# wavelab/libwave

Measured on AMD Instinct MI355X. Metric: point-cloud registrations/sec (1M<->1M pts, ICP), higher is better.
Workload: dtype f32

## Files before the change

include/wavematch.h:

```cpp
#ifndef WAVEMATCH_H
#define WAVEMATCH_H

#include <stddef.h>
#include <stdint.h>

#ifdef __cplusplus
extern "C" {
#endif

#define WM_OK 0
#define WM_NOT_CONVERGED 1
#define WM_TOO_FEW_CORRESPONDENCES 2
#define WM_ERR_ARG (-1)
#define WM_ERR_HIP (-2)
#define WM_ERR_RCCL (-3)
#define WM_ERR_STATE (-4)
#define WM_ERR_NOMEM (-5)

enum { WM_MEM_HOST = 0, WM_MEM_DEVICE = 1 };

typedef struct wm_ctx wm_ctx;

int wm_ctx_create(wm_ctx **out, int device);
void wm_ctx_destroy(wm_ctx *ctx);
// ... 94 lines not shown
int wm_icp_batch_match(wm_ctx *ctx, const wm_batch_item *items, int n_items, size_t stride_bytes,
                       int mem, const wm_icp_params *p, float res, int multiscale_steps,
                       int with_info, double *T_out, double *info_out, wm_icp_stats *stats,
                       int *status);

int wm_voxel_downsample_batch(wm_ctx *ctx, const wm_batch_item *items, int n_items, size_t stride_bytes,
                              int mem, float leaf, float *out_xyz, size_t cap_points, size_t *n_out);

int wm_voxel_downsample(wm_ctx *ctx, const void *pts, size_t n, size_t stride_bytes, int mem,
                        float leaf, void *out, size_t out_stride, int out_mem, size_t cap,
                        size_t *n_out);

int wm_transform_cloud(wm_ctx *ctx, const void *pts, size_t n, size_t stride_bytes, int mem,
                       const double T[16], void *out, size_t out_stride, int out_mem);

enum { WM_INFO_LUM = 0, WM_INFO_CENSI = 1, WM_INFO_LUMOLD = 2 };
int wm_icp_info(wm_ctx *ctx, int method, const double T_result[16], double lin_covar,
                double ang_covar, double max_corr, double info[36], int *degenerate);

int wm_debug_copy_bandwidth(wm_ctx *ctx, size_t bytes, int reps, double *gb_per_s);
int wm_debug_bins_sum(const double *x, size_t n, const unsigned *perm, double *out, long long limbs_out[3]);
int wm_debug_sort_pairs(wm_ctx *ctx, const void *keys, int key_bytes, size_t n, unsigned bits, unsigned *values_out);
int wm_debug_knn(wm_ctx *ctx, int which, int k, int32_t *idx_out, float *d2_out);
int wm_set_option(wm_ctx *ctx, const char *name, double value);
int wm_debug_cert_log(wm_ctx *ctx, int iterations, unsigned *out, int cap);
int wm_debug_cert_prof(wm_ctx *ctx, unsigned long long *out, int cap);
int wm_debug_pub_log(wm_ctx *ctx, unsigned long long *out, int cap);
int wm_get_iteration_times(wm_ctx *ctx, float *nn_ms, int cap);

int wm_debug_solve_cycles(wm_ctx *ctx, unsigned long long out[8]);
int wm_debug_cost_log(wm_ctx *ctx, int iterations, unsigned *out, size_t cap);
int wm_debug_phase_log(wm_ctx *ctx, unsigned long long *out, int iterations);

int wm_get_correspondences(wm_ctx *ctx, int32_t *match_idx, float *d2, size_t cap);

int wm_nn_search(wm_ctx *ctx, const double T[16], double max_corr, int nn_method,
                 int32_t *match_idx, float *d2, size_t cap, float *kernel_ms);

int wm_estimate_normals(wm_ctx *ctx, int which, int k, void *normals_out, int out_mem);

#define WM_STATS_LEN 32
int wm_icp_stats_for(wm_ctx *ctx, const double T[16], int mode, double stats[WM_STATS_LEN]);

int wm_debug_rank_select(wm_ctx *ctx, const float *vals, size_t n, size_t rank, float *out);

typedef struct { int n_matched, n_kept; float threshold_d2; int all_kept; } wm_icp_reject_result;
// ... 343 lines not shown
```

libwave_amd/capi.py:

```python
import ctypes as C
import os

import numpy as np

_HERE = os.path.dirname(os.path.abspath(__file__))
LIB_PATH = os.path.join(_HERE, "libwavematch_hip.so")

WM_OK, WM_NOT_CONVERGED, WM_TOO_FEW = 0, 1, 2
WM_ERR_ARG, WM_ERR_HIP, WM_ERR_RCCL, WM_ERR_STATE, WM_ERR_NOMEM = -1, -2, -3, -4, -5
WM_NDT_BATCH_MAX_POINTS = 200000
WM_GICP_BATCH_MAX_POINTS = 100000
WM_BATCH_LDS_TARGET_POINTS = 10000
WM_BATCH_MAX_TARGET_POINTS = 65535
WM_GROUND_BATCH_MAX_KEYS = 0xFFFFFFFF
WM_GROUND_BATCH_MAX_POINTS = 0x7FFFFFF0
WM_MEM_HOST, WM_MEM_DEVICE = 0, 1
WM_ICP_SVD, WM_ICP_GN6, WM_ICP_PLANE = 0, 1, 2
WM_REJECT_NONE, WM_REJECT_TRIMMED, WM_REJECT_MEDIAN = 0, 1, 2
WM_NN_AUTO, WM_NN_GRID, WM_NN_BRUTE = 0, 1, 2
WM_NN_WARM = 0x100
WM_INFO_LUM, WM_INFO_CENSI, WM_INFO_LUMOLD = 0, 1, 2
WM_STATS_LEN = 32
CONV_NAMES = {0: "NOT_CONVERGED", 1: "ITERATIONS", 2: "TRANSFORM", 3: "ABS_MSE", 4: "REL_MSE",
              5: "NO_CORRESPONDENCES", 6: "FORCED", 7: "DEGENERATE"}
# ... 287 lines not shown
        L.wm_comm_world.argtypes = [C.c_void_p]
        L.wm_comm_mailboxes.argtypes = [C.c_void_p]
        L.wm_comm_set_exchange_timeout_ms.argtypes = [C.c_void_p, C.c_int]
        L.wm_icp_align_sharded.argtypes = [C.c_void_p, C.c_void_p, C.c_void_p, C.c_size_t, C.c_void_p,
                                           C.c_size_t, C.c_size_t, C.c_int, C.POINTER(IcpParams), _dp,
                                           C.POINTER(IcpStats)]
        L.wm_ndt_set_comm.argtypes = [C.c_void_p, C.c_void_p]
        L.wm_ndt_build_model.argtypes = [C.c_void_p, C.c_double]
        L.wm_set_source_filtered.argtypes = [C.c_void_p, C.c_void_p, C.c_size_t, C.c_size_t, C.c_int, C.c_float]
        L.wm_set_target_filtered.argtypes = [C.c_void_p, C.c_void_p, C.c_size_t, C.c_size_t, C.c_int, C.c_float]
        L.wm_multi_create.argtypes = [C.POINTER(C.c_void_p), C.POINTER(C.c_int), C.c_int, C.c_int]
        L.wm_multi_destroy.argtypes = [C.c_void_p]
        L.wm_multi_destroy.restype = None
        L.wm_multi_size.argtypes = [C.c_void_p]
        L.wm_multi_icp_align.argtypes = [C.c_void_p, C.c_void_p, C.c_size_t, C.c_void_p, C.c_size_t,
                                         C.c_size_t, C.POINTER(IcpParams), _dp, C.POINTER(IcpStats)]
        L.wm_multi_icp_match.argtypes = [C.c_void_p, C.c_void_p, C.c_size_t, C.c_void_p, C.c_size_t,
                                         C.c_size_t, C.POINTER(IcpParams), C.c_float, C.c_int, _dp, C.POINTER(IcpStats)]
        L.wm_multi_icp_info.argtypes = [C.c_void_p, C.c_int, _dp, C.c_double, C.c_double, C.c_double, _dp,
                                        C.POINTER(C.c_int)]
        L.wm_debug_solve_cycles.argtypes = [C.c_void_p, C.POINTER(C.c_uint64)]
        L.wm_debug_sort_pairs.argtypes = [C.c_void_p, C.c_void_p, C.c_int, C.c_size_t, C.c_uint, C.c_void_p]
        L.wm_debug_knn.argtypes = [C.c_void_p, C.c_int, C.c_int, _ip, _fp]
        L.wm_debug_cost_log.argtypes = [C.c_void_p, C.c_int, C.c_void_p, C.c_size_t]
        L.wm_debug_phase_log.argtypes = [C.c_void_p, C.c_void_p, C.c_int]
        L.wm_get_correspondences.argtypes = [C.c_void_p, _ip, _fp, C.c_size_t]
        L.wm_nn_search.argtypes = [C.c_void_p, _dp, C.c_double, C.c_int, _ip, _fp, C.c_size_t, _fp]
        L.wm_icp_stats_for.argtypes = [C.c_void_p, _dp, C.c_int, _dp]
        L.wm_debug_rank_select.argtypes = [C.c_void_p, _fp, C.c_size_t, C.c_size_t, _fp]
        L.wm_icp_reject.argtypes = [C.c_void_p, _dp, C.c_int, C.c_int, C.c_double, C.c_double, C.c_int,
                                    C.POINTER(IcpRejectResult), C.c_void_p, _dp]
        L.wm_estimate_normals.argtypes = [C.c_void_p, C.c_int, C.c_int, C.c_void_p, C.c_int]
        L.wm_umeyama_from_stats.argtypes = [_dp, _dp]
        L.wm_gn6_from_stats.argtypes = [_dp, _dp]
        L.wm_ground_default_params.argtypes = [C.POINTER(GroundParams)]
        L.wm_ground_default_params.restype = None
        L.wm_ground_segment.argtypes = [C.c_void_p, C.c_void_p, C.c_size_t, C.c_size_t, C.c_int,
                                        C.POINTER(GroundParams), C.c_int, C.c_void_p, C.c_size_t, C.c_int,
                                        C.POINTER(C.c_size_t), C.c_void_p, C.POINTER(GroundStats)]
        L.wm_ground_segment_batch.argtypes = [C.c_void_p, C.POINTER(GroundScan), C.c_int, C.c_size_t, C.c_int,
                                              C.POINTER(GroundParams), C.c_int, C.c_void_p, C.c_size_t, C.c_void_p,
                                              C.c_size_t, C.c_int, C.POINTER(C.c_size_t), C.c_void_p,
                                              C.POINTER(GroundStats), C.POINTER(C.c_float)]
        L.wm_outlier_default_params.argtypes = [C.POINTER(OutlierParams)]
        L.wm_outlier_default_params.restype = None
        L.wm_outlier_filter.argtypes = [C.c_void_p, C.c_void_p, C.c_size_t, C.c_size_t, C.c_int, C.POINTER(OutlierParams),
# ... 1055 lines not shown
    def phase_log_fetch(self, iterations):
        buf = np.zeros((iterations, 8), np.uint64)
        k = lib().wm_debug_phase_log(self._h, buf.ctypes.data_as(C.c_void_p), iterations)
        return buf[:max(k, 0)]

    def sort_pairs(self, keys, bits):
        keys = np.ascontiguousarray(keys)
        assert keys.dtype in (np.uint32, np.uint64) and keys.ndim == 1
        out = np.zeros(keys.shape[0], np.uint32)
        self._check(lib().wm_debug_sort_pairs(self._h, keys.ctypes.data, keys.dtype.itemsize, keys.shape[0], int(bits),
                                              out.ctypes.data), "wm_debug_sort_pairs")
        return out

    def debug_knn(self, which, k):
        n = self.n_tgt if which == 1 else self.n_src
        idx = np.full((n, int(k)), -1, np.int32)
        d2 = np.zeros((n, int(k)), np.float32)
        rc = self._check(lib().wm_debug_knn(self._h, int(which), int(k), idx.ctypes.data_as(_ip), d2.ctypes.data_as(_fp)),
                         "wm_debug_knn")
        if rc != WM_OK:
            raise WmError("wm_debug_knn: %s" % lib().wm_strerror(rc).decode())
        return idx, d2

    def solve_cycles(self):
        buf = (C.c_uint64 * 8)()
        lib().wm_debug_solve_cycles(self._h, buf)
        return [int(v) for v in buf]

    def iteration_times(self, cap=1024):
        buf = np.zeros(cap, np.float32)
        n = lib().wm_get_iteration_times(self._h, buf.ctypes.data_as(_fp), cap)
        return buf[:n].copy()

    def correspondences(self):
        idx = np.empty(self.n_src, np.int32)
        d2 = np.empty(self.n_src, np.float32)
        self._check(lib().wm_get_correspondences(self._h, idx.ctypes.data_as(_ip),
                                                 d2.ctypes.data_as(_fp), self.n_src),
                    "wm_get_correspondences")
        return idx, d2

    def nn_search(self, T=None, max_corr=3.0, nn_method=WM_NN_AUTO, want=True, timed=False):
        T = np.ascontiguousarray(np.eye(4) if T is None else T, np.float64)
        idx = np.empty(self.n_src, np.int32) if want else None
        d2 = np.empty(self.n_src, np.float32) if want else None
        ms = C.c_float(0)
# ... 177 lines not shown
```

libwave_amd/csrc/wm_ctx.hip:

```cpp
#include "wm_internal.hpp"

#include <float.h>
#include <stdlib.h>
#include <string.h>

#include <new>

namespace wm {

int prepare_work(wm_ctx *ctx) {
    const size_t n = ctx->n_src > 0 ? ctx->n_src : 1;
    WM_HIP(ctx, ctx->keys.reserve(n * sizeof(unsigned long long)));
    WM_HIP(ctx, ctx->match_pt.reserve(n * sizeof(float4)));
    WM_HIP(ctx, ctx->partials.reserve((n / 64 + 1024) * kAcc * sizeof(double)));
    WM_HIP(ctx, ctx->d_state.reserve(sizeof(IcpDevState)));
    if (!ctx->h_state)
        WM_HIP(ctx, hipHostMalloc((void **) &ctx->h_state, sizeof(IcpDevState), hipHostMallocDefault));
    return WM_OK;
}

bool use_brute(const wm_ctx *ctx, int nn_method) {
    if (nn_method == WM_NN_BRUTE) return true;
    if (nn_method == WM_NN_GRID) return false;
    return (double) ctx->n_src * (double) ctx->n_tgt_input <= 4.0e6;
// ... 164 lines not shown
    {"nn_balanced", "WM_TUNE_NN_BALANCED", &wm_ctx::tune_nn_balanced, nullptr, kIntMin, kIntMax, 0},
    {"lag", "WM_TUNE_LAG", &wm_ctx::tune_lag, nullptr, 1, 16, 0},
    {"spin_us", "WM_TUNE_SPIN_US", &wm_ctx::tune_spin_us, nullptr, kIntMin, kIntMax, 0},
    {"cert_from", "WM_TUNE_CERT_FROM", &wm_ctx::tune_cert_from, nullptr, kIntMin, kIntMax, 0},
    {"cert_disp", "WM_TUNE_CERT_DISP", nullptr, &wm_ctx::tune_cert_disp, 0, kFloatMax, kOpenLo},
    {"cert_changed", "WM_TUNE_CERT_CHANGED", nullptr, &wm_ctx::tune_cert_changed, 0, kFloatMax, kOpenLo},
    {"cert_unsettled", "WM_TUNE_CERT_UNSETTLED", nullptr, &wm_ctx::tune_cert_unsettled, 0, kFloatMax, kOpenLo},
    {"cert_pad_mul", "WM_TUNE_CERT_PAD_MUL", nullptr, &wm_ctx::tune_cert_pad_mul, 0, kFloatMax, 0},
    {"cert_pad_frac", "WM_TUNE_CERT_PAD_FRAC", nullptr, &wm_ctx::tune_cert_pad_frac, 0, kFloatMax, 0},
    {"late", "WM_TUNE_LATE", &wm_ctx::tune_late, nullptr, kIntMin, kIntMax, kFlag},
    {"bins", "WM_TUNE_BINS", &wm_ctx::tune_bins, nullptr, kIntMin, kIntMax, 0},
    {"early_source", "WM_TUNE_EARLY_SOURCE", &wm_ctx::tune_early_source, nullptr, kIntMin, kIntMax, 0},
    {"shard_force", "WM_SHARD_FORCE", &wm_ctx::tune_force_shard, nullptr, kIntMin, kIntMax, 0},
    {"trace", "WM_TRACE", &wm_ctx::trace, nullptr, kIntMin, kIntMax, kFlag},
    {"gicp_served", "WM_TUNE_GICP_SERVED", &wm_ctx::tune_gicp_served, nullptr, kIntMin, 2, kFlag},
    {"gicp_serve_test_stall_ms", "WM_TUNE_GICP_SERVE_TEST_STALL_MS", &wm_ctx::gicp_serve_test_stall_ms, nullptr, kIntMin, kIntMax, 0},
    {"gicp_blocks", "WM_TUNE_GICP_BLOCKS", &wm_ctx::tune_gicp_blocks, nullptr, 1, 4096, 0},
    {"knn_r0", "WM_TUNE_KNN_R0", nullptr, &wm_ctx::tune_knn_r0, 0.25, 8, kOrZero},
    {"gicp_profile", "WM_GICP_PROFILE", &wm_ctx::gicp_profile, nullptr, kIntMin, kIntMax, kFlag},
    {"outlier_cell_div", "WM_TUNE_OUTLIER_CELL_DIV", nullptr, &wm_ctx::tune_outlier_cell_div, 0.5, 8, 0},
    {"cluster_cell_div", "WM_TUNE_CLUSTER_CELL_DIV", nullptr, &wm_ctx::tune_cluster_cell_div, 0.5, 8, 0},
    {"sac_round", "WM_TUNE_SAC_ROUND", &wm_ctx::tune_sac_round, nullptr, 1, 1024, 0},
    {"radix_min", "WM_TUNE_RADIX_MIN", &wm_ctx::tune_radix_min, nullptr, kIntMin, kIntMax, 0},
    {"ndt_dense", "WM_TUNE_NDT_DENSE", &wm_ctx::tune_ndt_dense, nullptr, kIntMin, kIntMax, 0},
    {"ndt_vox_split", "WM_TUNE_NDT_VOX_SPLIT", &wm_ctx::tune_ndt_vox_split, nullptr, kIntMin, kIntMax, kNdtModel},
    {"ndt_keys64", "WM_TUNE_NDT_KEYS64", &wm_ctx::tune_ndt_keys64, nullptr, kIntMin, kIntMax, kFlag | kNdtModel},
    {"ndt_blocks", "WM_TUNE_NDT_BLOCKS", &wm_ctx::tune_ndt_blocks, nullptr, 0, 4096, 0},
    {"ndt_spec_hessian", "WM_TUNE_NDT_SPEC_HESSIAN", &wm_ctx::tune_ndt_spec_hessian, nullptr, kIntMin, kIntMax, 0},
    {"ndt_fused_fetch", "WM_TUNE_NDT_FUSED_FETCH", &wm_ctx::tune_ndt_fused_fetch, nullptr, kIntMin, kIntMax, 0},
    {"ndt_profile", "WM_NDT_PROFILE", &wm_ctx::ndt_profile, nullptr, kIntMin, kIntMax, kFlag},
};

int apply_option(wm_ctx *ctx, const Option &o, double v) {
    if ((o.flags & kFlag) && v != o.hi) v = v != 0 ? 1 : 0;
    if ((!(v >= o.lo && v <= o.hi) || ((o.flags & kOpenLo) && v == o.lo)) && !((o.flags & kOrZero) && v == 0)) return WM_ERR_ARG;
    if (o.i) ctx->*o.i = (int) v;
    else ctx->*o.f = (float) v;
    if (o.flags & kNdtModel) ctx->ndt_built = false;
    return WM_OK;
}
}

int wm_set_option(wm_ctx *ctx, const char *name, double value) {
    if (!ctx || !name) return WM_ERR_ARG;
    for (const Option &o : kOptions)
        if (strcmp(name, o.name) == 0) return apply_option(ctx, o, value);
// ... 31 lines not shown

int wm_ctx_set_stream(wm_ctx *ctx, void *hip_stream, int external) {
    if (!ctx) return WM_ERR_ARG;
    WM_HIP(ctx, hipSetDevice(ctx->device));
    WM_HIP(ctx, hipStreamSynchronize(ctx->stream));
    ctx->stream = external ? static_cast<hipStream_t>(hip_stream) : ctx->own_stream;
    return WM_OK;
}

void wm_ctx_destroy(wm_ctx *ctx) {
    if (!ctx) return;
    (void) hipSetDevice(ctx->device);
    if (ctx->stream) (void) hipStreamSynchronize(ctx->stream);
    DevBuf *bufs[] = {&ctx->src_sorted, &ctx->tgt_orig, &ctx->staging, &ctx->staging2, &ctx->cell_of, &ctx->counts,
                      &ctx->block_sums, &ctx->bbox_buf, &ctx->cloud_bbox, &ctx->keys, &ctx->keys_bak, &ctx->match_pt, &ctx->match_pt_bak, &ctx->d_levels, &ctx->ndt_keys, &ctx->ndt_keys2,
                      &ctx->ndt_vox, &ctx->ndt_vkey, &ctx->ndt_hkeys, &ctx->ndt_hvals, &ctx->ndt_dense, &ctx->ndt_meanf, &ctx->src_orig,
                      &ctx->gicp_c1, &ctx->gicp_c2, &ctx->gicp_mahal, &ctx->gicp_mailbox, &ctx->src_grid.pts,
                      &ctx->src_grid.cell_start, &ctx->vg_idx, &ctx->vg_idx2, &ctx->vg_perm,
                      &ctx->vg_perm2, &ctx->vg_tmp, &ctx->vg_seg, &ctx->io_a, &ctx->io_b, &ctx->ds_ref,
                      &ctx->ds_tgt, &ctx->match_ref, &ctx->match_tgt,
                      &ctx->partials, &ctx->partials2, &ctx->bins, &ctx->nn_bound, &ctx->late_ctl, &ctx->cert_count, &ctx->cert_prof, &ctx->cost_log, &ctx->phase_log, &ctx->shard_ref, &ctx->shard_tgt,
                      &ctx->shard_ref_band, &ctx->shard_tgt_band, &ctx->shard_misc, &ctx->shard_flags, &ctx->shard_pos_t,
                      &ctx->shard_pos_s, &ctx->shard_stats, &ctx->ndt_sum_dev, &ctx->corr_tmp_idx, &ctx->corr_tmp_d2, &ctx->d_state,
                      &ctx->plane_nrm, &ctx->plane_nrm_src, &ctx->plane_bins, &ctx->reject_buf, &ctx->reject_tmp};
    for (DevBuf *b : bufs) b->release();
    ctx->icp_stage.release();
    ctx->gicp_stage.release();
    ctx->ndt_stage.release();
    batch_voxel_release(ctx);
    ground_release(ctx);
    outlier_release(ctx);
    cluster_release(ctx);
    sac_release(ctx);
    boxes_release(ctx);
    fpfh_release(ctx);
    for (auto &l : ctx->levels) {
        l.pts.release();
        l.cell_start.release();
    }
    if (ctx->h_state) (void) hipHostFree(ctx->h_state);
    if (ctx->h_gicp) (void) hipHostFree(ctx->h_gicp);
    if (ctx->h_gicp_slots) (void) hipHostFree(ctx->h_gicp_slots);
    if (ctx->h_ndt) (void) hipHostFree(ctx->h_ndt);
    if (ctx->h_sig) (void) hipHostFree(ctx->h_sig);
    if (ctx->h_pub) (void) hipHostFree(ctx->h_pub);
    if (ctx->h_late) (void) hipHostFree(ctx->h_late);
    if (ctx->ev_block) (void) hipEventDestroy(ctx->ev_block);
// ... 102 lines not shown
```

libwave_amd/csrc/wm_debug.hip:

```cpp
#include "wm_internal.hpp"
#include "wm_bins.hpp"

#include <algorithm>
#include <vector>

#include <math.h>

namespace wm {

void late_debug_report(wm_ctx *ctx, unsigned late_blocks, int inside, int reason) {
    unsigned long long d[64 * 4];
    (void) hipStreamSynchronize(ctx->stream);
    if (hipMemcpy(d, (char *) ctx->late_ctl.p + late_ctl_bytes(), sizeof(d), hipMemcpyDeviceToHost) == hipSuccess) {
        fprintf(stderr, "[wm] late kernel: %d iterations, reason %d\n", inside, reason);
        for (int k = 0; k < inside && k < 64; ++k)
            fprintf(stderr, "  it %2d: workers (hand-out -> all rows in) %6.2f us | rows added %5.2f | solve %5.2f | hand-out %5.2f\n", k,
                    k ? ((long long) d[k * 4] - (long long) d[(k - 1) * 4 + 3]) * 0.01 : 0.0,
                    (d[k * 4 + 1] - d[k * 4]) * 0.01, (d[k * 4 + 2] - d[k * 4 + 1]) * 0.01,
                    (d[k * 4 + 3] - d[k * 4 + 2]) * 0.01);
        const int li = ctx->late_debug_iter;
        std::vector<unsigned long long> wst((size_t) late_blocks * 8);
        if (li >= 1 && li < inside && li < 64 && ctx->cert_prof.p &&
            hipMemcpy(wst.data(), ctx->cert_prof.p, wst.size() * 8, hipMemcpyDeviceToHost) == hipSuccess) {
            const unsigned long long t0 = d[(li - 1) * 4 + 3];
// ... 117 lines not shown
    for (int i = 0; i < n; ++i) {
        unsigned t = 0;
        for (int k = 0; k < 64; ++k) t += tmp[(size_t) i * 64 + k];
        out[i] = t;
    }
    return n;
}

int wm_debug_pub_log(wm_ctx *ctx, unsigned long long *out, int cap) {
    if (!ctx || !out || !ctx->h_pub) return WM_ERR_ARG;
    const int n = ctx->h_pub_slots < cap ? ctx->h_pub_slots : cap;
    for (int k = 0; k < n; ++k) out[k] = ctx->h_pub[k];
    return n;
}

int wm_debug_cert_prof(wm_ctx *ctx, unsigned long long *out, int cap) {
    if (!ctx || !out || !ctx->cert_prof.p) return WM_ERR_ARG;
    WM_HIP(ctx, hipSetDevice(ctx->device));
    const int n = ctx->cert_log_iter < cap ? ctx->cert_log_iter : cap;
    if (n > 0) WM_TRY(copy_to_caller(ctx, out, ctx->cert_prof.p, (size_t) n * 64 * sizeof(unsigned long long)));
    return n;
}

int wm_get_iteration_times(wm_ctx *ctx, float *nn_ms, int cap) {
    if (!ctx || !nn_ms || cap < 0) return 0;
    int n = (int) ctx->iter_nn_ms.size();
    if (n > cap) n = cap;
    for (int i = 0; i < n; ++i) nn_ms[i] = ctx->iter_nn_ms[i];
    return n;
}

}
```

libwave_amd/csrc/wm_grid.hip:

```cpp
#include <cstring>

#include <rocprim/rocprim.hpp>

#include "wm_internal.hpp"
#include "wm_sort.hpp"

#include <math.h>
#include <vector>
#include <string.h>

namespace wm {

__global__ void __launch_bounds__(kBlock) k_pack(const unsigned char *in, size_t n, size_t stride,
                                                  float4 *out) {
    size_t i = (size_t) blockIdx.x * kBlock + threadIdx.x;
    if (i >= n) return;
    const float *p = reinterpret_cast<const float *>(in + i * stride);
    float x = p[0], y = p[1], z = p[2];
    if (!(isfinite(x) && isfinite(y) && isfinite(z))) {
        x = y = z = __builtin_nanf("");
    }
    out[i] = make_float4(x, y, z, __uint_as_float((unsigned) i));
}

// ... 162 lines not shown
        for (int d = 0; d < 3; ++d) {
            out->lo[d] = lo[d];
            out->hi[d] = hi[d];
        }
}

int compute_bbox(wm_ctx *ctx, const float4 *pts, size_t n, Bbox *out, size_t *n_valid) {
    for (int d = 0; d < 3; ++d) out->lo[d] = out->hi[d] = 0.f;
    *n_valid = 0;
    if (n == 0) return WM_OK;
    float *res = (float *) pinned_scratch(ctx, 8 * sizeof(float) * kBboxBlocks);
    if (!res) return WM_ERR_HIP;
    WM_HIP(ctx, ctx->bbox_buf.reserve(8 * sizeof(float) * kBboxBlocks));
    unsigned blocks = 0;
    WM_TRY(launch_bbox(ctx, pts, n, ctx->bbox_buf.as<float>(), &blocks));
    WM_TRY(fast_fetch(ctx, res, ctx->bbox_buf.p, 8 * sizeof(float) * blocks));
    finish_bbox(res, blocks, out, n_valid);
    return WM_OK;
}

struct LinearKey {
    float ox, oy, oz, inv_h;
    int nx, ny, nz;
    __device__ unsigned operator()(const float4 &p) const {
        int cx = (int) floorf((p.x - ox) * inv_h);
        int cy = (int) floorf((p.y - oy) * inv_h);
        int cz = (int) floorf((p.z - oz) * inv_h);
        cx = min(max(cx, 0), nx - 1);
        cy = min(max(cy, 0), ny - 1);
        cz = min(max(cz, 0), nz - 1);
        return (unsigned) ((cz * ny + cy) * nx + cx);
    }
};

__device__ inline unsigned spread3(unsigned v) {
    v &= 0x3FFu;
    v = (v | (v << 16)) & 0x030000FFu;
    v = (v | (v << 8)) & 0x0300F00Fu;
    v = (v | (v << 4)) & 0x030C30C3u;
    v = (v | (v << 2)) & 0x09249249u;
    return v;
}

struct MortonKey {
    float ox, oy, oz, sx, sy, sz;
    int cells;
    __device__ unsigned operator()(const float4 &p) const {
        int cx = min(max((int) ((p.x - ox) * sx), 0), cells - 1);
        int cy = min(max((int) ((p.y - oy) * sy), 0), cells - 1);
        int cz = min(max((int) ((p.z - oz) * sz), 0), cells - 1);
        return spread3((unsigned) cx) | (spread3((unsigned) cy) << 1) |
               (spread3((unsigned) cz) << 2);
    }
};
// ... 52 lines not shown
    WM_HIP(ctx, hipGetLastError());
    return WM_OK;
}

template <class KeyFn>
static int counting_sort(wm_ctx *ctx, const float4 *pts, size_t n, KeyFn key, size_t ncells,
                         unsigned *cell_start , float4 *out) {
    WM_HIP(ctx, ctx->cell_of.reserve(2 * n * sizeof(unsigned)));
    WM_HIP(ctx, ctx->counts.reserve(ncells * sizeof(unsigned)));
    unsigned *counts = ctx->counts.as<unsigned>();
    unsigned *cell_of = ctx->cell_of.as<unsigned>(), *rank_of = cell_of + n;
    WM_HIP(ctx, hipMemsetAsync(counts, 0, ncells * sizeof(unsigned), ctx->stream));
    unsigned blocks = (unsigned) ((n + kBlock - 1) / kBlock);
    hipLaunchKernelGGL(HIP_KERNEL_NAME(k_count<KeyFn>), dim3(blocks), dim3(kBlock), 0, ctx->stream,
                       pts, n, key, cell_of, rank_of, counts);
    WM_HIP(ctx, hipGetLastError());
    WM_TRY(exclusive_scan(ctx, counts, ncells, cell_start));
    hipLaunchKernelGGL(k_scatter, dim3(blocks), dim3(kBlock), 0, ctx->stream, pts, n, cell_of, rank_of,
                       cell_start, out, ncells);
    WM_HIP(ctx, hipGetLastError());
    return WM_OK;
}

constexpr int kOccBlocks = 1024;
__global__ void __launch_bounds__(kBlock) k_count_occupied(const unsigned *cell_start,
                                                            size_t ncells, unsigned *out) {
    unsigned c = 0;
    for (size_t i = (size_t) blockIdx.x * kBlock + threadIdx.x; i < ncells;
         i += (size_t) gridDim.x * kBlock)
        c += (cell_start[i + 1] != cell_start[i]);
    for (int off = 32; off > 0; off >>= 1) c += __shfl_down(c, off);
    __shared__ unsigned s_c[kBlock / 64];
    if ((threadIdx.x & 63) == 0) s_c[threadIdx.x >> 6] = c;
    __syncthreads();
    if (threadIdx.x == 0) {
        for (int w = 1; w < kBlock / 64; ++w) c += s_c[w];
        out[blockIdx.x] = c;
    }
}

__global__ void k_pad_tail(const unsigned *cell_start, size_t ncells, float4 *pts) {
    const unsigned end = cell_start[ncells];
    const float nanv = __builtin_nanf("");
    if (threadIdx.x < 4) pts[end + threadIdx.x] = make_float4(nanv, nanv, nanv, __uint_as_float(kNoIdx));
}

static void grid_dims(const Bbox &bb, float h, int *nx, int *ny, int *nz) {
    *nx = (int) floor((bb.hi[0] - bb.lo[0]) / h) + 1;
    *ny = (int) floor((bb.hi[1] - bb.lo[1]) / h) + 1;
    *nz = (int) floor((bb.hi[2] - bb.lo[2]) / h) + 1;
}

int build_grid_level(wm_ctx *ctx, const float4 *pts, size_t n, const Bbox &bb, float h,
                     GridLevel *lvl, double *avg_occupancy) {
    int nx, ny, nz;
    grid_dims(bb, h, &nx, &ny, &nz);
    uint64_t ncells = (uint64_t) nx * ny * nz;
    lvl->ncells = ncells;
    WM_HIP(ctx, lvl->pts.reserve((n + 4) * sizeof(float4)));
    WM_HIP(ctx, lvl->cell_start.reserve((ncells + 1) * sizeof(unsigned)));
    LinearKey key{bb.lo[0], bb.lo[1], bb.lo[2], 1.0f / h, nx, ny, nz};
    if (n > 0) {
        WM_TRY(counting_sort(ctx, pts, n, key, ncells, lvl->cell_start.as<unsigned>(),
                             lvl->pts.as<float4>()));
    } else {
        WM_HIP(ctx, hipMemsetAsync(lvl->cell_start.p, 0, (ncells + 1) * sizeof(unsigned),
                                   ctx->stream));
        hipLaunchKernelGGL(k_pad_tail, dim3(1), dim3(64), 0, ctx->stream, lvl->cell_start.as<unsigned>(),
                           (size_t) ncells, lvl->pts.as<float4>());
    }
    float extent = fmaxf(fmaxf(bb.hi[0] - bb.lo[0], bb.hi[1] - bb.lo[1]), bb.hi[2] - bb.lo[2]);
    float amax = 0;
    for (int d = 0; d < 3; ++d) amax = fmaxf(amax, fmaxf(fabsf(bb.lo[d]), fabsf(bb.hi[d])));
    float ulp = fmaxf(amax, extent) * 1.2e-7f;
    lvl->d.ox = bb.lo[0];
    lvl->d.oy = bb.lo[1];
    lvl->d.oz = bb.lo[2];
    lvl->d.h = h;
    lvl->d.inv_h = 1.0f / h;
    lvl->d.slack = fmaxf(1e-3f, 8.0f * ulp / h);
    lvl->d.nx = nx;
    lvl->d.ny = ny;
    lvl->d.nz = nz;
    lvl->d.pts = lvl->pts.as<float4>();
    lvl->d.cell_start = lvl->cell_start.as<unsigned>();
// ... 106 lines not shown
    unsigned total = 0;
#pragma unroll
    for (int r = 0; r < 4; ++r) {
        unsigned s, e;
        child_run(fs, fnx, fny, fnz, X, Y, Z, r, &s, &e);
        total += e - s;
    }
    counts[c] = total;
}

__global__ void __launch_bounds__(kBlock)
    k_coarse_move(const unsigned *__restrict__ fs, const float4 *__restrict__ fpts, size_t fncells,
                  LinearKey key0, int shift, int fnx, int fny, int fnz, int cnx, int cny,
                  const unsigned *__restrict__ cs, float4 *__restrict__ out, size_t cncells) {
    const unsigned j = blockIdx.x * kBlock + threadIdx.x;
    if (j == 0) {
        const unsigned end = cs[(size_t) cncells];
        const float nanv = __builtin_nanf("");
#pragma unroll
        for (int u = 0; u < 4; ++u) out[end + u] = make_float4(nanv, nanv, nanv, __uint_as_float(kNoIdx));
    }
    if (j >= fs[fncells]) return;
    const float4 p = fpts[j];
    int x = min(max((int) floorf((p.x - key0.ox) * key0.inv_h), 0), key0.nx - 1) >> shift;
    int y = min(max((int) floorf((p.y - key0.oy) * key0.inv_h), 0), key0.ny - 1) >> shift;
    int z = min(max((int) floorf((p.z - key0.oz) * key0.inv_h), 0), key0.nz - 1) >> shift;
    const int X = x >> 1, Y = y >> 1, Z = z >> 1, r = (y & 1) + 2 * (z & 1);
    unsigned dst = cs[((size_t) Z * cny + Y) * cnx + X];
    for (int q = 0; q < r; ++q) {
        unsigned s, e;
        child_run(fs, fnx, fny, fnz, X, Y, Z, q, &s, &e);
        dst += e - s;
    }
    unsigned s, e;
    child_run(fs, fnx, fny, fnz, X, Y, Z, r, &s, &e);
    out[dst + (j - s)] = p;
}

static int derive_grid_level(wm_ctx *ctx, const GridLevel &fine, int fine_index, GridLevel *lvl,
                             size_t n) {
    const GridDev &f = fine.d;
    const int nx = (f.nx + 1) / 2, ny = (f.ny + 1) / 2, nz = (f.nz + 1) / 2;
    const uint64_t ncells = (uint64_t) nx * ny * nz;
    lvl->ncells = ncells;
    WM_HIP(ctx, lvl->pts.reserve((n + 4) * sizeof(float4)));
    WM_HIP(ctx, lvl->cell_start.reserve((ncells + 1) * sizeof(unsigned)));
    WM_HIP(ctx, ctx->counts.reserve(ncells * sizeof(unsigned)));
    unsigned *counts = ctx->counts.as<unsigned>();
    const unsigned blocks = (unsigned) ((ncells + kBlock - 1) / kBlock);
// ... 139 lines not shown
```

libwave_amd/csrc/wm_internal.hpp:

```cpp
#pragma once
#include <stdio.h>

#include <hip/hip_runtime.h>
#include <stdint.h>

#include <chrono>
#include <string>
#include <thread>
#include <vector>

#include "../../include/wavematch.h"
#include "wm_math.hpp"

namespace wm {

constexpr int kMaxLevels = 6;
constexpr int kBlock = 256;
constexpr unsigned kNoIdx = 0xFFFFFFFFu;
constexpr int kBlkLen = 34;
constexpr int kAcc = 18;

#define WM_HIP(ctx, call)                                                              \
    do {                                                                               \
        hipError_t _e = (call);                                                        \
// ... 211 lines not shown
    float tune_r_light = 16.0f;
    int tune_xcd_chunk = 32;
    int tune_nn_balanced = 1;
    int tune_lag = 2;
    int tune_spin_us = 80;
    int tune_bins = 1;
    int tune_early_source = 2;
    int tune_force_shard = 0;
    int tune_cert_from = -1;
    float tune_cert_disp = 0.15f;
    float tune_cert_changed = 0.05f;
    float tune_cert_unsettled = 0.40f;
    float tune_cert_pad_mul = 8.f, tune_cert_pad_frac = 0.5f;
    int tune_late = 0;
    int tune_gicp_served = 1;
    int gicp_serve_test_stall_ms = 0;
    int tune_gicp_blocks = 256;
    float tune_knn_r0 = 0.f;
    int gicp_profile = 0;
    float tune_outlier_cell_div = 2.f;
    float tune_cluster_cell_div = 2.f;
    int tune_sac_round = 256;
    int tune_radix_min = 256 << 10;
    int tune_ndt_dense = 2;
    int tune_ndt_vox_split = -1;
    int tune_ndt_keys64 = 0;
    int tune_ndt_blocks = 0;
    int tune_ndt_spec_hessian = 1;
    int tune_ndt_fused_fetch = 1;
    int ndt_profile = 0;
    int late_debug_iter = -1;
    bool cert_prof_on = false;
    std::string gicp_trace_path;
    bool gicp_serve_debug = false;
    int gicp_small_trace = 0;

    double tuned_h = 0, tuned_vol = 0;
    size_t tuned_n = 0;
    double tuned_src_h = 0, tuned_src_vol = 0;
    unsigned tuned_src_uses = 0;
    size_t tuned_src_n = 0;

    wm::DevBuf staging, staging2, cell_of, counts, block_sums, bbox_buf;
    wm::DevBuf match_pt, match_pt_bak;
    wm::PairStage icp_stage, gicp_stage, ndt_stage;
    void *batch_voxel = nullptr;
    void *ground = nullptr;
    void *outlier = nullptr;
    void *cluster = nullptr;
    void *sac = nullptr;
    void *boxes = nullptr;
    void *fpfh = nullptr;
    wm::DevBuf phase_log;
    wm::DevBuf cost_log;
    int cost_log_iter = 0, cost_log_cap = 0;
    wm::DevBuf keys, partials, partials2, corr_tmp_idx, corr_tmp_d2, d_levels;
    wm::LevelsDev levels_dev{};
    wm::DevBuf bins;
    bool bins_dirty = false;
    wm::DevBuf nn_bound;
    wm::DevBuf cert_count;
    wm::DevBuf cert_prof;
    int cert_log_iter = 0, cert_log_cap = 0;
    int cert_launches = 0;
    int late_capacity = 0;
    wm::DevBuf late_ctl;
// ... 260 lines not shown
```

Measured before the change: 294.3.

## Build grid levels with a two-pass row-band counting sort

Adds a new grid-construction path that first bins points into bands of (z,y) rows using per-tile LDS histograms, scans them, and scatters points into band order. A per-band kernel then does a cell-level counting sort in LDS to produce cell_start and the sorted points. The goal is to replace the global per-cell counting sort with LDS-local atomics, reducing global atomics and scan work over large cell counts. It is enabled by default through tune_grid_rows=1 when the grid shape and size fit the limits, and it costs an extra temporary buffer plus an extra pass over the points. A debug API for dumping grid levels is also added.

```diff
diff --git a/include/wavematch.h b/include/wavematch.h
--- a/include/wavematch.h
+++ b/include/wavematch.h
@@ -140,6 +140,8 @@
 int wm_debug_bins_sum(const double *x, size_t n, const unsigned *perm, double *out, long long limbs_out[3]);
 int wm_debug_sort_pairs(wm_ctx *ctx, const void *keys, int key_bytes, size_t n, unsigned bits, unsigned *values_out);
 int wm_debug_knn(wm_ctx *ctx, int which, int k, int32_t *idx_out, float *d2_out);
+int wm_debug_grid_level(wm_ctx *ctx, int level, double max_corr, float geom[5], int dims[3], size_t *n_points,
+                        unsigned *cell_start, size_t cell_cap, float *pts, size_t pts_cap);
 int wm_set_option(wm_ctx *ctx, const char *name, double value);
 int wm_debug_cert_log(wm_ctx *ctx, int iterations, unsigned *out, int cap);
 int wm_debug_cert_prof(wm_ctx *ctx, unsigned long long *out, int cap);
diff --git a/libwave_amd/capi.py b/libwave_amd/capi.py
--- a/libwave_amd/capi.py
+++ b/libwave_amd/capi.py
@@ -333,6 +333,8 @@
         L.wm_debug_solve_cycles.argtypes = [C.c_void_p, C.POINTER(C.c_uint64)]
         L.wm_debug_sort_pairs.argtypes = [C.c_void_p, C.c_void_p, C.c_int, C.c_size_t, C.c_uint, C.c_void_p]
         L.wm_debug_knn.argtypes = [C.c_void_p, C.c_int, C.c_int, _ip, _fp]
+        L.wm_debug_grid_level.argtypes = [C.c_void_p, C.c_int, C.c_double, _fp, _ip, C.POINTER(C.c_size_t), C.c_void_p,
+                                          C.c_size_t, C.c_void_p, C.c_size_t]
         L.wm_debug_cost_log.argtypes = [C.c_void_p, C.c_int, C.c_void_p, C.c_size_t]
         L.wm_debug_phase_log.argtypes = [C.c_void_p, C.c_void_p, C.c_int]
         L.wm_get_correspondences.argtypes = [C.c_void_p, _ip, _fp, C.c_size_t]
@@ -1434,6 +1436,20 @@
             raise WmError("wm_debug_knn: %s" % lib().wm_strerror(rc).decode())
         return idx, d2
 
+    def debug_grid_level(self, level, max_corr=0.0):
+        geom = np.zeros(5, np.float32)
+        dims = np.zeros(3, np.int32)
+        n = C.c_size_t(0)
+        args = (self._h, int(level), float(max_corr), geom.ctypes.data_as(_fp), dims.ctypes.data_as(_ip), C.byref(n))
+        self._check(lib().wm_debug_grid_level(*args, None, 0, None, 0), "wm_debug_grid_level")
+        ncells = int(dims[0]) * int(dims[1]) * int(dims[2])
+        cell_start = np.zeros(ncells + 1, np.uint32)
+        pts = np.zeros((n.value + 4, 4), np.float32)
+        self._check(lib().wm_debug_grid_level(*args, cell_start.ctypes.data, cell_start.size, pts.ctypes.data, pts.shape[0]),
+                    "wm_debug_grid_level")
+        return dict(origin=geom[:3].copy(), h=geom[3], inv_h=geom[4], dims=tuple(int(d) for d in dims),
+                    cell_start=cell_start, pts=pts)
+
     def solve_cycles(self):
         buf = (C.c_uint64 * 8)()
         lib().wm_debug_solve_cycles(self._h, buf)
diff --git a/libwave_amd/csrc/wm_ctx.hip b/libwave_amd/csrc/wm_ctx.hip
--- a/libwave_amd/csrc/wm_ctx.hip
+++ b/libwave_amd/csrc/wm_ctx.hip
@@ -210,6 +210,7 @@
     {"cluster_cell_div", "WM_TUNE_CLUSTER_CELL_DIV", nullptr, &wm_ctx::tune_cluster_cell_div, 0.5, 8, 0},
     {"sac_round", "WM_TUNE_SAC_ROUND", &wm_ctx::tune_sac_round, nullptr, 1, 1024, 0},
     {"radix_min", "WM_TUNE_RADIX_MIN", &wm_ctx::tune_radix_min, nullptr, kIntMin, kIntMax, 0},
+    {"grid_rows", "WM_TUNE_GRID_ROWS", &wm_ctx::tune_grid_rows, nullptr, 0, 2, 0},
     {"ndt_dense", "WM_TUNE_NDT_DENSE", &wm_ctx::tune_ndt_dense, nullptr, kIntMin, kIntMax, 0},
     {"ndt_vox_split", "WM_TUNE_NDT_VOX_SPLIT", &wm_ctx::tune_ndt_vox_split, nullptr, kIntMin, kIntMax, kNdtModel},
     {"ndt_keys64", "WM_TUNE_NDT_KEYS64", &wm_ctx::tune_ndt_keys64, nullptr, kIntMin, kIntMax, kFlag | kNdtModel},
@@ -287,7 +288,8 @@
                       &ctx->partials, &ctx->partials2, &ctx->bins, &ctx->nn_bound, &ctx->late_ctl, &ctx->cert_count, &ctx->cert_prof, &ctx->cost_log, &ctx->phase_log, &ctx->shard_ref, &ctx->shard_tgt,
                       &ctx->shard_ref_band, &ctx->shard_tgt_band, &ctx->shard_misc, &ctx->shard_flags, &ctx->shard_pos_t,
                       &ctx->shard_pos_s, &ctx->shard_stats, &ctx->ndt_sum_dev, &ctx->corr_tmp_idx, &ctx->corr_tmp_d2, &ctx->d_state,
-                      &ctx->plane_nrm, &ctx->plane_nrm_src, &ctx->plane_bins, &ctx->reject_buf, &ctx->reject_tmp};
+                      &ctx->plane_nrm, &ctx->plane_nrm_src, &ctx->plane_bins, &ctx->reject_buf, &ctx->reject_tmp,
+                      &ctx->row_hist, &ctx->row_tmp};
     for (DevBuf *b : bufs) b->release();
     ctx->icp_stage.release();
     ctx->gicp_stage.release();
diff --git a/libwave_amd/csrc/wm_debug.hip b/libwave_amd/csrc/wm_debug.hip
--- a/libwave_amd/csrc/wm_debug.hip
+++ b/libwave_amd/csrc/wm_debug.hip
@@ -163,6 +163,28 @@
     return n;
 }
 
+int wm_debug_grid_level(wm_ctx *ctx, int level, double max_corr, float geom[5], int dims[3], size_t *n_points,
+                        unsigned *cell_start, size_t cell_cap, float *pts, size_t pts_cap) {
+    if (!ctx || level < 0 || level >= kMaxLevels || !geom || !dims || !n_points) return WM_ERR_ARG;
+    if (ctx->n_tgt_input == 0) return WM_ERR_STATE;
+    WM_HIP(ctx, hipSetDevice(ctx->device));
+    if (max_corr > 0) {
+        WM_TRY(finalize_clouds(ctx));
+        WM_TRY(ensure_levels(ctx, max_corr));
+    }
+    if (level >= ctx->n_levels || !ctx->levels[level].built) return WM_ERR_STATE;
+    const GridLevel &l = ctx->levels[level];
+    geom[0] = l.d.ox, geom[1] = l.d.oy, geom[2] = l.d.oz, geom[3] = l.d.h, geom[4] = l.d.inv_h;
+    dims[0] = l.d.nx, dims[1] = l.d.ny, dims[2] = l.d.nz;
+    unsigned total = 0;
+    WM_TRY(copy_to_caller(ctx, &total, l.cell_start.as<unsigned>() + l.ncells, sizeof(unsigned)));
+    *n_points = total;
+    if ((cell_start && cell_cap < l.ncells + 1) || (pts && pts_cap < (size_t) total + 4)) return WM_ERR_ARG;
+    if (cell_start) WM_TRY(copy_to_caller(ctx, cell_start, l.cell_start.p, (l.ncells + 1) * sizeof(unsigned)));
+    if (pts) WM_TRY(copy_to_caller(ctx, pts, l.pts.p, ((size_t) total + 4) * sizeof(float4)));
+    return WM_OK;
+}
+
 int wm_get_iteration_times(wm_ctx *ctx, float *nn_ms, int cap) {
     if (!ctx || !nn_ms || cap < 0) return 0;
     int n = (int) ctx->iter_nn_ms.size();
diff --git a/libwave_amd/csrc/wm_grid.hip b/libwave_amd/csrc/wm_grid.hip
--- a/libwave_amd/csrc/wm_grid.hip
+++ b/libwave_amd/csrc/wm_grid.hip
@@ -208,14 +208,21 @@
 struct LinearKey {
     float ox, oy, oz, inv_h;
     int nx, ny, nz;
+    __device__ void cell(const float4 &p, int *cx, int *cy, int *cz) const {
+        *cx = min(max((int) floorf((p.x - ox) * inv_h), 0), nx - 1);
+        *cy = min(max((int) floorf((p.y - oy) * inv_h), 0), ny - 1);
+        *cz = min(max((int) floorf((p.z - oz) * inv_h), 0), nz - 1);
+    }
+    __device__ void row_x(const float4 &p, unsigned *row, unsigned *cx) const {
+        int x, y, z;
+        cell(p, &x, &y, &z);
+        *row = (unsigned) (z * ny + y);
+        *cx = (unsigned) x;
+    }
     __device__ unsigned operator()(const float4 &p) const {
-        int cx = (int) floorf((p.x - ox) * inv_h);
-        int cy = (int) floorf((p.y - oy) * inv_h);
-        int cz = (int) floorf((p.z - oz) * inv_h);
-        cx = min(max(cx, 0), nx - 1);
-        cy = min(max(cy, 0), ny - 1);
-        cz = min(max(cz, 0), nz - 1);
-        return (unsigned) ((cz * ny + cy) * nx + cx);
+        unsigned row, cx;
+        row_x(p, &row, &cx);
+        return row * (unsigned) nx + cx;
     }
 };
 
@@ -314,6 +321,183 @@
     return WM_OK;
 }
 
+constexpr int kRowThreads = 512;
+constexpr int kRowTile = kRowThreads * 8;
+constexpr unsigned kRowNxCap = 4000;
+constexpr unsigned kRowCounterWords = 16000;
+constexpr unsigned kRowBandRows = 8;
+constexpr unsigned kRowMaxBands = 8192;
+constexpr uint64_t kRowMaxTable = 1ull << 22;
+
+__device__ __forceinline__ unsigned rows_lds_scan(unsigned *a, unsigned n, unsigned *s_wave) {
+    const unsigned tid = threadIdx.x, lane = tid & 63u, wave = tid >> 6;
+    const unsigned per = (n + kRowThreads - 1) / kRowThreads;
+    const unsigned b = min(tid * per, n), e = min(b + per, n);
+    unsigned sum = 0;
+    for (unsigned i = b; i < e; ++i) sum += a[i];
+    const unsigned incl = wave_incl_scan(sum, lane);
+    if (lane == 63u) s_wave[wave] = incl;
+    __syncthreads();
+    unsigned run = incl - sum, all = 0;
+    for (unsigned w = 0; w < (unsigned) (kRowThreads / 64); ++w) {
+        if (w < wave) run += s_wave[w];
+        all += s_wave[w];
+    }
+    for (unsigned i = b; i < e; ++i) {
+        const unsigned v = a[i];
+        a[i] = run;
+        run += v;
+    }
+    __syncthreads();
+    return all;
+}
+
+__global__ void __launch_bounds__(kRowThreads) k_rows_hist(const float4 *__restrict__ pts, unsigned n, LinearKey key, unsigned rshift,
+                                                            unsigned bands, unsigned tiles, unsigned *__restrict__ hist) {
+    extern __shared__ unsigned s_mem[];
+    const unsigned tid = threadIdx.x, tile = blockIdx.x;
+    for (unsigned b = tid; b < bands; b += kRowThreads) s_mem[b] = 0u;
+    __syncthreads();
+    float4 p[8];
+#pragma unroll
+    for (unsigned r = 0; r < 8u; ++r) {
+        const unsigned i = tile * (unsigned) kRowTile + r * kRowThreads + tid;
+        p[r] = i < n ? pts[i] : make_float4(NAN, 0.f, 0.f, 0.f);
+    }
+#pragma unroll
+    for (unsigned r = 0; r < 8u; ++r)
+        if (p[r].x == p[r].x) {
+            unsigned row, cx;
+            key.row_x(p[r], &row, &cx);
+            atomicAdd(&s_mem[row >> rshift], 1u);
+        }
+    __syncthreads();
+    for (unsigned b = tid; b < bands; b += kRowThreads) hist[(size_t) b * tiles + tile] = s_mem[b];
+}
+
+__global__ void __launch_bounds__(kRowThreads) k_rows_scatter(const float4 *__restrict__ pts, unsigned n, LinearKey key, unsigned rshift,
+                                                               unsigned bands, unsigned tiles, const unsigned *__restrict__ hist,
+                                                               const unsigned *__restrict__ totals, unsigned *__restrict__ band_start,
+                                                               float4 *__restrict__ tmp) {
+    extern __shared__ unsigned s_mem[];
+    __shared__ unsigned s_wave[kRowThreads / 64];
+    const unsigned tid = threadIdx.x, tile = blockIdx.x;
+    float4 p[8];
+#pragma unroll
+    for (unsigned r = 0; r < 8u; ++r) {
+        const unsigned i = tile * (unsigned) kRowTile + r * kRowThreads + tid;
+        p[r] = i < n ? pts[i] : make_float4(NAN, 0.f, 0.f, 0.f);
+    }
+    for (unsigned b = tid; b < bands; b += kRowThreads) s_mem[b] = totals[b];
+    __syncthreads();
+    const unsigned all = rows_lds_scan(s_mem, bands, s_wave);
+    if (tile == 0) {
+        for (unsigned b = tid; b < bands; b += kRowThreads) band_start[b] = s_mem[b];
+        if (tid == 0) band_start[bands] = all;
+    }
+    for (unsigned b = tid; b < bands; b += kRowThreads) s_mem[b] += hist[(size_t) b * tiles + tile];
+    __syncthreads();
+#pragma unroll
+    for (unsigned r = 0; r < 8u; ++r)
+        if (p[r].x == p[r].x) {
+            unsigned row, cx;
+            key.row_x(p[r], &row, &cx);
+            tmp[atomicAdd(&s_mem[row >> rshift], 1u)] = p[r];
+        }
+}
+
+__global__ void __launch_bounds__(kRowThreads) k_rows_finish(const float4 *__restrict__ tmp, const unsigned *__restrict__ band_start,
+                                                              LinearKey key, unsigned nrows, unsigned rshift,
+                                                              unsigned *__restrict__ cell_start, float4 *__restrict__ out) {
+    extern __shared__ unsigned s_mem[];
+    __shared__ unsigned s_wave[kRowThreads / 64];
+    const unsigned nx = (unsigned) key.nx, tid = threadIdx.x;
+    const unsigned r0 = blockIdx.x << rshift;
+    const unsigned cells = min(1u << rshift, nrows - r0) * nx;
+    const unsigned s = band_start[blockIdx.x], e = band_start[blockIdx.x + 1];
+    for (unsigned k = tid; k < cells; k += kRowThreads) s_mem[k] = 0u;
+    __syncthreads();
+    for (unsigned j0 = s + tid; j0 < e; j0 += 4u * kRowThreads) {
+        float4 p[4];
+#pragma unroll
+        for (unsigned u = 0; u < 4u; ++u) {
+            const unsigned j = j0 + u * kRowThreads;
+            p[u] = j < e ? tmp[j] : make_float4(NAN, 0.f, 0.f, 0.f);
+        }
+#pragma unroll
+        for (unsigned u = 0; u < 4u; ++u)
+            if (j0 + u * kRowThreads < e) {
+                unsigned row, cx;
+                key.row_x(p[u], &row, &cx);
+                atomicAdd(&s_mem[min((row - r0) * nx + cx, cells - 1u)], 1u);
+            }
+    }
+    __syncthreads();
+    if (e != s) rows_lds_scan(s_mem, cells, s_wave);
+    unsigned *cs = cell_start + (size_t) r0 * nx;
+    for (unsigned k = tid; k < cells; k += kRowThreads) cs[k] = s + s_mem[k];
+    if (blockIdx.x == gridDim.x - 1 && tid == 0) {
+        cs[cells] = e;
+        const float nanv = __builtin_nanf("");
+#pragma unroll
+        for (int u = 0; u < 4; ++u) out[e + u] = make_float4(nanv, nanv, nanv, __uint_as_float(kNoIdx));
+    }
+    __syncthreads();
+    for (unsigned j0 = s + tid; j0 < e; j0 += 4u * kRowThreads) {
+        float4 p[4];
+#pragma unroll
+        for (unsigned u = 0; u < 4u; ++u) {
+            const unsigned j = j0 + u * kRowThreads;
+            p[u] = j < e ? tmp[j] : make_float4(NAN, 0.f, 0.f, 0.f);
+        }
+#pragma unroll
+        for (unsigned u = 0; u < 4u; ++u)
+            if (j0 + u * kRowThreads < e) {
+                unsigned row, cx;
+                key.row_x(p[u], &row, &cx);
+                out[s + atomicAdd(&s_mem[min((row - r0) * nx + cx, cells - 1u)], 1u)] = p[u];
+            }
+    }
+}
+
+constexpr unsigned kRowMinRows = 2048, kRowMinPoints = 32768;
+static bool rows_apply(int option, int nx, int ny, int nz, size_t n, unsigned *rshift) {
+    if (option == 0 || n == 0 || (unsigned) nx > kRowNxCap) return false;
+    const uint64_t nrows = (uint64_t) ny * nz;
+    unsigned sh = 0;
+    while ((2u << sh) <= kRowBandRows && (2u << sh) * (unsigned) nx <= kRowCounterWords) ++sh;
+    while (((nrows - 1) >> sh) + 1 > kRowMaxBands && (2u << sh) * (unsigned) nx <= kRowCounterWords) ++sh;
+    const uint64_t bands = ((nrows - 1) >> sh) + 1, tiles = (n + kRowTile - 1) / kRowTile;
+    if (bands > kRowMaxBands || bands * tiles > kRowMaxTable) return false;
+    *rshift = sh;
+    if (option == 2) return true;
+    return nx >= 3 && nrows >= kRowMinRows && n >= kRowMinPoints;
+}
+static_assert(kRowCounterWords / kRowNxCap >= 1 && kRowCounterWords * sizeof(unsigned) + 64 <= 65536, "k_rows_finish's LDS");
+
+static int counting_sort_rows(wm_ctx *ctx, const float4 *pts, size_t n, const LinearKey &key, unsigned rshift,
+                              unsigned *cell_start , float4 *out) {
+    const unsigned nrows = (unsigned) key.ny * (unsigned) key.nz;
+    const unsigned bands = ((nrows - 1) >> rshift) + 1, tiles = (unsigned) ((n + kRowTile - 1) / kRowTile);
+    WM_HIP(ctx, ctx->row_tmp.reserve(n * sizeof(float4)));
+    WM_HIP(ctx, ctx->row_hist.reserve(((size_t) bands * tiles + 2 * (size_t) bands + 1) * sizeof(unsigned)));
+    unsigned *hist = ctx->row_hist.as<unsigned>(), *totals = hist + (size_t) bands * tiles, *band_start = totals + bands;
+    float4 *tmp = ctx->row_tmp.as<float4>();
+    const size_t band_lds = (size_t) bands * sizeof(unsigned);
+    hipLaunchKernelGGL(k_rows_hist, dim3(tiles), dim3(kRowThreads), band_lds, ctx->stream, pts, (unsigned) n, key, rshift, bands, tiles, hist);
+    WM_HIP(ctx, hipGetLastError());
+    hipLaunchKernelGGL(k_rs_scan, dim3(bands), dim3(kRsThreads), 0, ctx->stream, hist, tiles, totals);
+    WM_HIP(ctx, hipGetLastError());
+    hipLaunchKernelGGL(k_rows_scatter, dim3(tiles), dim3(kRowThreads), band_lds, ctx->stream, pts, (unsigned) n, key, rshift, bands, tiles,
+                       (const unsigned *) hist, (const unsigned *) totals, band_start, tmp);
+    WM_HIP(ctx, hipGetLastError());
+    const size_t cell_lds = ((size_t) key.nx << rshift) * sizeof(unsigned);
+    hipLaunchKernelGGL(k_rows_finish, dim3(bands), dim3(kRowThreads), cell_lds, ctx->stream, (const float4 *) tmp,
+                       (const unsigned *) band_start, key, nrows, rshift, cell_start, out);
+    WM_HIP(ctx, hipGetLastError());
+    return WM_OK;
+}
+
 constexpr int kOccBlocks = 1024;
 __global__ void __launch_bounds__(kBlock) k_count_occupied(const unsigned *cell_start,
                                                             size_t ncells, unsigned *out) {
@@ -352,7 +536,10 @@
     WM_HIP(ctx, lvl->pts.reserve((n + 4) * sizeof(float4)));
     WM_HIP(ctx, lvl->cell_start.reserve((ncells + 1) * sizeof(unsigned)));
     LinearKey key{bb.lo[0], bb.lo[1], bb.lo[2], 1.0f / h, nx, ny, nz};
-    if (n > 0) {
+    unsigned rshift = 0;
+    if (rows_apply(ctx->tune_grid_rows, nx, ny, nz, n, &rshift)) {
+        WM_TRY(counting_sort_rows(ctx, pts, n, key, rshift, lvl->cell_start.as<unsigned>(), lvl->pts.as<float4>()));
+    } else if (n > 0) {
         WM_TRY(counting_sort(ctx, pts, n, key, ncells, lvl->cell_start.as<unsigned>(),
                              lvl->pts.as<float4>()));
     } else {
@@ -505,9 +692,11 @@
     }
     if (j >= fs[fncells]) return;
     const float4 p = fpts[j];
-    int x = min(max((int) floorf((p.x - key0.ox) * key0.inv_h), 0), key0.nx - 1) >> shift;
-    int y = min(max((int) floorf((p.y - key0.oy) * key0.inv_h), 0), key0.ny - 1) >> shift;
-    int z = min(max((int) floorf((p.z - key0.oz) * key0.inv_h), 0), key0.nz - 1) >> shift;
+    int x, y, z;
+    key0.cell(p, &x, &y, &z);
+    x >>= shift;
+    y >>= shift;
+    z >>= shift;
     const int X = x >> 1, Y = y >> 1, Z = z >> 1, r = (y & 1) + 2 * (z & 1);
     unsigned dst = cs[((size_t) Z * cny + Y) * cnx + X];
     for (int q = 0; q < r; ++q) {
diff --git a/libwave_amd/csrc/wm_internal.hpp b/libwave_amd/csrc/wm_internal.hpp
--- a/libwave_amd/csrc/wm_internal.hpp
+++ b/libwave_amd/csrc/wm_internal.hpp
@@ -257,6 +257,7 @@
     float tune_cluster_cell_div = 2.f;
     int tune_sac_round = 256;
     int tune_radix_min = 256 << 10;
+    int tune_grid_rows = 1;
     int tune_ndt_dense = 2;
     int tune_ndt_vox_split = -1;
     int tune_ndt_keys64 = 0;
@@ -277,6 +278,7 @@
     size_t tuned_src_n = 0;
 
     wm::DevBuf staging, staging2, cell_of, counts, block_sums, bbox_buf;
+    wm::DevBuf row_hist, row_tmp;
     wm::DevBuf match_pt, match_pt_bak;
     wm::PairStage icp_stage, gicp_stage, ndt_stage;
     void *batch_voxel = nullptr;
```

Result: faster. 299.4, median of 6 (+1.7%).
